# prstrive/SuRF

Measured on AMD Instinct MI355X. Metric: rays/sec (576x800, 5-view, 128 samp/ray render, whole job), higher is better.
Workload: dtype f32 (operands split exactly into 3 bf16 pieces, fp32 accumulate)

## Files before the change

surf_amd/csrc/sdf_mlp_split.hip:

```cpp
#include <math.h>
#include <stdlib.h>
#include <string.h>

#include "common.h"

#include "sdf_split_common.h"

namespace {

#ifdef SURF_SDF_TIMING
__device__ unsigned long long g_phase[8];
#define SURF_T(k)                                                 \
  do {                                                            \
    const unsigned long long now_ = __builtin_readcyclecounter(); \
    c.tacc[k] += now_ - c.tprev;                                  \
    c.tprev = now_;                                               \
  } while (0)
#else
#define SURF_T(k)
#endif

struct Ctx {
#ifdef SURF_SDF_TIMING
  mutable unsigned long long tprev;
  mutable unsigned long long tacc[8];
#endif
  rsrc_t wr, sr, sl, tr;
  int lane, lane16, h, svoff, wave;
  int wave1024;
  int dma_voff;
  uint32_t dma_lds;
  char* lds;
  char* lds_s;
  u32x4 I0, I1;
};
__device__ __forceinline__ u32x4 minus_identity_frag(int lane, int s) {
  const int i = lane & 31, g = lane >> 5;
  u32x4 f = {0u, 0u, 0u, 0u};
#pragma unroll
  for (int ip = 0; ip < 8; ++ip) {
    const int rho = (ip & 3) + 8 * (2 * s + (ip >> 2)) + 4 * g;
    if (rho == i) f[ip >> 1] |= (ip & 1) ? 0xBF800000u : 0x0000BF80u;
  }
  return f;
}
template <class P>
__device__ __forceinline__ void mres_step(const Ctx& c, f32x16& vt, const u32x4& piece, int s2) {
  if constexpr (P::MRES) {
    __builtin_amdgcn_sched_barrier(0);
    const u32x4 I = s2 ? c.I1 : c.I0;
    vt = __builtin_amdgcn_mfma_f32_32x32x16_bf16(__builtin_bit_cast(bf16x8, I), __builtin_bit_cast(bf16x8, piece), vt, 0, 0, 0);
    asm volatile("" ::"v"(vt));
    __builtin_amdgcn_sched_barrier(0);
  }
}

template <class P> constexpr int n_dma(int ci) { return (P::CH.ks[ci] * P::NP + 3) / 4; }
#ifndef SURF_SDF_DMA_WAVEMAJOR
#define SURF_SDF_DMA_WAVEMAJOR 1
#endif
template <class P, int NS, int CI, int k>
__device__ __forceinline__ void stage_dma_piece(const Ctx& c) {
  constexpr int OFF = P::CH.off[CI];
#if SURF_SDF_DMA_WAVEMAJOR
  constexpr int ND = n_dma<P>(CI);
  const uint32_t wshare = (uint32_t)c.wave1024 * (uint32_t)ND;
  __builtin_amdgcn_raw_ptr_buffer_load_lds(
      c.wr, (__attribute__((address_space(3))) void*)(uintptr_t)(c.dma_lds + wshare + ((CI % NS) * slot_bytes<P>() + (k >> 2) * 4096)), 16,
      c.lane16, (int)wshare + (OFF + (k >> 2) * 4096), (k & 3) * 1024, 0);
#else
  __builtin_amdgcn_raw_ptr_buffer_load_lds(
      c.wr, (__attribute__((address_space(3))) void*)(uintptr_t)(c.dma_lds + ((CI % NS) * slot_bytes<P>() + k * 4096)), 16, c.dma_voff,
      OFF + k * 4096, 0, 0);
#endif
}
template <class P, int NS, int CI, int K = 0>
__device__ __forceinline__ void stage_dma(const Ctx& c) {
  if constexpr (K < n_dma<P>(CI)) {
    stage_dma_piece<P, NS, CI, K>(c);
    stage_dma<P, NS, CI, K + 1>(c);
  }
}
constexpr int sprime_layer(bool deep, int L, int T, bool r0 = false) {
  if (!deep) return (L >= 1 && T < 4) ? L - 1 : -1;
  if (L >= 1 && T < 3) return L - 1;
  if (r0 && L == 2 && T == BWD_NT[L] - 1) return -1;
  if (L >= 2 && T == BWD_NT[L] - 1) return L - 2;
  return -1;
}
constexpr int sprime_tile(bool deep, int L, int T) { return !deep ? T : ((L >= 1 && T < 3) ? T + 1 : 0); }
template <class P> constexpr int lds_slice(int layer, int tile) {
  const int k = (4 - layer) * 4 + tile;
  return (layer <= 4 && layer >= 0 && k < P::LDS_SLICES) ? k : -1;
}
template <class P> constexpr int reg_slice(int layer, int tile) {
  const int k = (4 - layer) * 4 + tile - P::LDS_SLICES;
  return (layer <= 4 && layer >= 0 && k >= 0 && k < P::REG_SLICES) ? k : -1;
}
template <class P> constexpr bool on_chip(int layer, int tile) {
  return lds_slice<P>(layer, tile) >= 0 || reg_slice<P>(layer, tile) >= 0 || (P::R0 && layer == 0);
}
template <class P> struct RegSlices {
  f32x4 v[P::REG_SLICES > 0 ? P::REG_SLICES : 1][4];
  f32x16 r0[P::R0 ? 4 : 1];
};
constexpr int sprime_groups(int layer, int tile) { return (layer == 2 && tile == 3) ? 2 : 4; }
template <class P> constexpr int vm_pre(int ci) {
  if (ci < N_FWD_CHUNKS) return (ci / 4 == 5 && ci % 4 > 0) ? 4 : 0;
  if (ci >= P::CH.n) return 0;
  if (P::R0 && ci == r0_chunk()) return 0;
  int l = 5, t = ci - N_FWD_CHUNKS - ((P::R0 && ci > r0_chunk()) ? 1 : 0);
  while (t >= BWD_NT[l]) { t -= BWD_NT[l]; --l; }
  if (l == 0) return P::DEEPJ ? 12 : 0;
  if (sprime_layer(P::DEEP, l, t, P::R0) < 0 || on_chip<P>(sprime_layer(P::DEEP, l, t, P::R0), sprime_tile(P::DEEP, l, t))) return 0;
  return sprime_groups(sprime_layer(P::DEEP, l, t, P::R0), sprime_tile(P::DEEP, l, t));
}
template <class P, bool GRAD> constexpr int vm_post(int ci) {
  if (!GRAD || ci >= N_FWD_CHUNKS) return 0;
  const int l = ci / 4, t = ci % 4;
  if ((l == 0 && t == 0) || (l == 5 && t > 0)) return 0;
  return on_chip<P>(t == 0 ? l - 1 : l, t == 0 ? 3 : t - 1) ? 0 : 4;
}
template <class P, bool GRAD, int CI, int NCH>
constexpr int barrier_vmcnt() {
  constexpr int DIST = P::nslot(GRAD) - 1;
  int n = 0;
  for (int j = 0; j + 1 < DIST; ++j) {
    const int cj = (CI - j + NCH) % NCH;
    n += vm_pre<P>(cj) + n_dma<P>((cj + DIST) % NCH) + vm_post<P, GRAD>(cj);
  }
  return n;
}
template <class P, bool GRAD, int CI, int NCH>
__device__ __forceinline__ void stage_barrier() {
  constexpr int N = barrier_vmcnt<P, GRAD, CI, NCH>();
  static_assert(N >= 0 && N < 64, "vmcnt");
  asm volatile("; surf_ring_window %1\n\ts_waitcnt vmcnt(%0) lgkmcnt(0)\n\ts_barrier" ::"n"(N), "n"(P::nslot(GRAD) - 2) : "memory");
}

template <class P, bool GRAD, int CI, int NCH, class PL, int NACC, class BSel, class F>
__device__ __forceinline__ void run_chunk_n(const Ctx& c, BSel bsel, F slot, f32x16 (&result)[NACC]) {
  constexpr int NKS = P::CH.ks[CI];
  constexpr int NP = P::NP, NM = P::NM;
  constexpr int NS = P::nslot(GRAD);
  constexpr int KPA = NKS > 0 ? NKS / NACC : 1;
  static_assert(NKS % NACC == 0, "k-steps per accumulator");
  const char* rd = c.lds + (CI % NS) * slot_bytes<P>() + c.lane16;
  typename P::Acc accs[NACC];
#pragma unroll
  for (int a = 0; a < NACC; ++a)
#pragma unroll
    for (int q = 0; q < P::NA; ++q)
#pragma unroll
      for (int r = 0; r < 16; ++r) accs[a].v[q][r] = 0.f;
  constexpr int PF = P::PF;
  static_assert(PF == 1, "the gap plan places the reads of k-step ks + 1 behind the MFMAs of k-step ks");
  u32x4 a_q[PF + 1][NP];
#pragma unroll
  for (int d = 0; d < PF; ++d)
#pragma unroll
    for (int p = 0; p < NP; ++p)
      if (d < NKS) a_q[d][p] = *reinterpret_cast<const u32x4*>(rd + (d * NP + p) * 1024);
  constexpr int NXT = (CI + NS - 1) % NCH, ND = n_dma<P>(NXT);
  static_assert(ND <= MAX_DMA && NKS * NM <= MAX_GAPS, "GapPlan sizes");
// ... 252 lines not shown
  mini_add_split(mp, P::NP, P::FUSED_SUB, P::MRES);
  return mp;
}
template <class P, int L, int T, bool CONVERT>
struct BwdPlan {
  static constexpr int CI = bwd_chunk(L, T, P::R0), NKS = P::CH.ks[CI];
  static constexpr MiniProg mini = bwd_prog<P>();
  static constexpr SlotProg prog = CONVERT ? weave(mini, 8, 0, P::MRES ? P::NP : 0) : SlotProg{};
  static constexpr GapPlan v = plan_gaps(NKS, P::NM, P::NP, chunk_dma<P, true, CI, n_chunks<P>(true)>(), NKS * P::NM, prog);
  static_assert(plan_ok(v, prog, mini, NKS * P::NM, NKS * P::NM), "gap plan");
};
template <class P, int L, int T, bool CONVERT>
__device__ __forceinline__ f32x16 bwd_tile(const Ctx& c, const FragT<P::NP>* din, FragT<P::NP>* dout, const BwdPend& prev,
                                           f32x4 (&s_load)[4], const RegSlices<P>& keep) {
  typedef FragT<P::NP> Frag;
  typedef BwdPlan<P, L, T, CONVERT> PL;
  constexpr int CI = bwd_chunk(L, T, P::R0);
  constexpr int SL = sprime_layer(P::DEEP, L, T, P::R0);
  constexpr int NG = SL >= 0 ? sprime_groups(SL, sprime_tile(P::DEEP, L, T)) : 0;
  static_assert((SL >= 0 && on_chip<P>(SL, sprime_tile(P::DEEP, L, T)) ? 0 : NG) + ((L == 0 && P::DEEPJ) ? 12 : 0) == vm_pre<P>(CI),
                "vmcnt bookkeeping");
  if (SL >= 0) load_sprime<P, NG>(c, SL, sprime_tile(P::DEEP, L, T), s_load, keep);
  MiniState<P::NP> st[2] = {};
  f32x16 vt = prev.G;
  auto slot = [&](auto sc) __attribute__((always_inline)) {
    constexpr int s = decltype(sc)::value;
    constexpr float inv_w = 1.0f / Scales<P>::W;
    constexpr int q = PL::prog.q[s] < 0 ? 0 : PL::prog.q[s], kind = PL::prog.kind[s], i = PL::prog.arg[s], el = 2 * q;
    MiniState<P::NP>& S = st[q & 1];
    if constexpr (kind == K_EXPN) {
      const f32x2 u = {prev.s[el >> 2][el & 3], prev.s[(el + 1) >> 2][(el + 1) & 3]};
      S.e[0] = SURF_X_NOSOFTPLUS ? u[0] : __builtin_amdgcn_exp2f(-u[0]);
      S.e[1] = SURF_X_NOSOFTPLUS ? u[1] : __builtin_amdgcn_exp2f(-u[1]);
      slot_pin(S.e);
    } else if constexpr (kind == K_ADD1) {
      slot_pin(S.e);
      S.d[0] = S.e[0] + 1.0f;
      S.d[1] = S.e[1] + 1.0f;
      slot_pin(S.d);
    } else if constexpr (kind == K_RCP) {
      slot_pin(S.d);
      S.r[0] = SURF_X_NOSOFTPLUS ? S.d[0] : __builtin_amdgcn_rcpf(S.d[0]);
      S.r[1] = SURF_X_NOSOFTPLUS ? S.d[1] : __builtin_amdgcn_rcpf(S.d[1]);
      slot_pin(S.r);
    } else if constexpr (kind == K_MULG) {
      slot_pin(S.r);
      S.val[0] = S.r[0] * (P::MRES ? vt[el] : prev.G[el]);
      S.val[1] = S.r[1] * (P::MRES ? vt[el + 1] : prev.G[el + 1]);
      if (inv_w != 1.0f) {
        S.val[0] *= inv_w;
        S.val[1] *= inv_w;
      }
      slot_pin(S.val);
    } else if constexpr (kind == K_PACK) {
      slot_pin(S.val);
      S.pc[i] = SURF_X_NOSPLIT ? __builtin_bit_cast(uint32_t, S.val[i & 1]) : P::pack(S.val);
      slot_pin(S.pc[i]);
      if (P::MRES) {
        dout[2 * (T - 1) + (el >> 3)].p[0][(el & 7) >> 1] = S.pc[0];
        vt[el] = S.val[0];
        vt[el + 1] = S.val[1];
      } else if (i == P::NP - 1) {
        Frag& f = dout[2 * (T - 1) + (el >> 3)];
#pragma unroll
        for (int k = 0; k < P::NP; ++k) f.p[k][(el & 7) >> 1] = S.pc[k];
      }
    } else if constexpr (kind == K_MRES) {
      mres_step<P>(c, vt, dout[2 * (T - 1) + (i & 1)].p[i >> 1], i & 1);
    } else if constexpr (kind == K_PACKT) {
      const f32x2 r2 = {vt[el], vt[el + 1]};
      dout[2 * (T - 1) + (el >> 3)].p[i][(el & 7) >> 1] = P::pack(r2);
    } else if constexpr (kind == K_EXPAND) {
      slot_pin(S.pc[i]);
      S.x = SURF_X_NOSPLIT ? S.val : P::expand(S.pc[i]);
      slot_pin(S.x);
    } else if constexpr (kind == K_SUB) {
      slot_pin(S.val, S.x);
      S.val[0] -= S.x[0];
      S.val[1] -= S.x[1];
      slot_pin(S.val);
    } else if constexpr (kind == K_SUBP) {
      S.val = SURF_X_NOSPLIT ? S.val : P::sub_piece(S.val, S.pc[i]);
    }
  };
  return run_chunk<P, true, CI, n_chunks<P>(true), PL>(
      c, [&](int ks) __attribute__((always_inline)) -> const Frag& { return din[ks]; }, slot);
}
template <class P, int L, int T>
__device__ __forceinline__ void bwd_hidden_tile(const Ctx& c, const FragT<P::NP>* din, FragT<P::NP>* dout, BwdPend& pend, const RegSlices<P>& keep) {
  const BwdPend prev = pend;
  f32x4 s_load[4] = {};
  const f32x16 G = bwd_tile<P, L, T, (T > 0)>(c, din, dout, prev, s_load, keep);
  pend.G = G;
#pragma unroll
  for (int g = 0; g < 4; ++g) {
    if (P::DEEP) {
      pend.s[g] = prev.sn[g];
      pend.sn[g] = s_load[g];
    } else {
      pend.s[g] = s_load[g];
    }
  }
}
template <class P, int L>
__device__ __forceinline__ void bwd_layer(const Ctx& c, const FragT<P::NP>* din, FragT<P::NP>* dout, f32x16& accE,
                                          f32x16& accP, BwdPend& pend, const RegSlices<P>& keep) {
  bwd_hidden_tile<P, L, 0>(c, din, dout, pend, keep);
  bwd_hidden_tile<P, L, 1>(c, din, dout, pend, keep);
  bwd_hidden_tile<P, L, 2>(c, din, dout, pend, keep);
  bwd_hidden_tile<P, L, 3>(c, din, dout, pend, keep);
  const BwdPend prev = pend;
  if constexpr (L == 3) {
    f32x4 unused[4];
    accE += bwd_tile<P, L, 4, true>(c, din, dout, prev, unused, keep);
    accP += bwd_tile<P, L, 5, false>(c, din, dout, prev, pend.sn, keep);
  } else {
    accP += bwd_tile<P, L, 4, true>(c, din, dout, prev, pend.sn, keep);
  }
}

template <class P, int CI>
struct R0Plan {
  static constexpr GapPlan v = plan_gaps(R0_KS, P::NM, P::NP, chunk_dma<P, true, CI, n_chunks<P>(true)>(), R0_KS * P::NM, SlotProg{});
};
template <class P>
__device__ __forceinline__ void recompute_layer0(const Ctx& c, const FragT<P::NP> (&ef)[2], RegSlices<P>& keep) {
  if constexpr (P::R0) {
    constexpr int CI = r0_chunk();
    static_assert(P::CH.ks[CI] == R0_KS && P::CH.off[CI] == P::CH.off[fwd_chunk(0, 0)] && fwd_ne(0) == 2 && fwd_nl(0) == 2, "R0 chunk");
    run_chunk_n<P, true, CI, n_chunks<P>(true), R0Plan<P, CI>, 4>(
        c, [&](int ks) __attribute__((always_inline)) -> const FragT<P::NP>& { return ef[ks & 1]; }, [&](auto) __attribute__((always_inline)) {},
        keep.r0);
  }
}

template <class P, int CI>
struct PadPlan {
  static constexpr GapPlan v = plan_gaps(0, P::NM, P::NP, chunk_dma<P, true, CI, n_chunks<P>(true)>(), 0, SlotProg{});
};
template <class P, int CI>
__device__ __forceinline__ void pad_chunks(const Ctx& c, const FragT<P::NP>* any) {
  if constexpr (CI < n_chunks<P>(true)) {
    run_chunk<P, true, CI, n_chunks<P>(true), PadPlan<P, CI>>(
        c, [&](int ks) __attribute__((always_inline)) -> const FragT<P::NP>& { return any[0]; }, [&](auto) __attribute__((always_inline)) {});
    pad_chunks<P, CI + 1>(c, any);
  }
}

template <class P, bool GRAD, bool BRICK = false>
__global__ __launch_bounds__(WPB * 64, P::occ(GRAD)) void sdf_mlp_split_kernel(SdfArgs a) {
  typedef FragT<P::NP> Frag;
  constexpr int NS = P::nslot(GRAD), NCH = n_chunks<P>(GRAD);
  constexpr int NSL = GRAD ? P::LDS_SLICES : 0;
  __shared__ __attribute__((aligned(16))) char lds[NS * slot_bytes<P>() + WPB * NSL * 4096];
  static_assert(NCH % NS == 0 && (!GRAD || NCH - P::CH.n <= MAX_PAD) && NS >= 3, "slot of a chunk = index % ring length");
  Ctx c;
  c.lane = threadIdx.x & 63;
  c.wave = __builtin_amdgcn_readfirstlane(threadIdx.x >> 6);
  c.h = c.lane >> 5;
  c.lane16 = c.lane * 16;
  c.lds = lds;
  c.lds_s = lds + NS * slot_bytes<P>() + c.wave * (NSL * 4096) + c.lane16;
  if (P::MRES) {
    c.I0 = minus_identity_frag(c.lane, 0);
    c.I1 = minus_identity_frag(c.lane, 1);
  }
  c.wave1024 = c.wave * 1024;
  c.dma_voff = c.lane16 + c.wave * 1024;
  c.dma_lds = (uint32_t)(uintptr_t)(__attribute__((address_space(3))) char*)lds + (SURF_SDF_DMA_WAVEMAJOR ? 0 : c.wave * 1024);
  c.wr = __builtin_amdgcn_make_buffer_rsrc((void*)a.packed, 0, stream_bytes<P>(), 0x00020000);
  c.tr = __builtin_amdgcn_make_buffer_rsrc((void*)(a.packed + stream_bytes<P>()), 0, TAIL_FLOATS * 4, 0x00020000);
  c.sr = __builtin_amdgcn_make_buffer_rsrc((void*)a.scratch, 0, (GRAD && !(SURF_X_NOSCRATCH & 1)) ? 0x7fffffff : 0, 0x00020000);
  c.sl = __builtin_amdgcn_make_buffer_rsrc((void*)a.scratch, 0, (GRAD && !(SURF_X_NOSCRATCH & 2)) ? 0x7fffffff : 0, 0x00020000);
  const int64_t wave_id = (int64_t)blockIdx.x * WPB + c.wave;
  c.svoff = (int)(wave_id * (SCR_SLOT * 4)) + c.lane * 16;
  const int64_t n_pts = a.n_dev ? (int64_t)*a.n_dev : a.n;
  const int64_t n_tiles = (n_pts + TILE - 1) / TILE;
  const int64_t n_rounds = (n_tiles + WPB - 1) / WPB;

  stage_dma<P, NS, 0>(c);
  stage_dma<P, NS, 1>(c);
  if (NS > 3) stage_dma<P, NS, 2>(c);
  if (NS > 4) stage_dma<P, NS, 3>(c);
  asm volatile("s_waitcnt vmcnt(0) lgkmcnt(0)\n\ts_barrier" ::: "memory");
#ifdef SURF_SDF_TIMING
  c.tprev = __builtin_readcyclecounter();
  for (int k = 0; k < 8; ++k) c.tacc[k] = 0;
#endif
  for (int64_t round = blockIdx.x; round < n_rounds; round += gridDim.x) {
    asm volatile("" : "+s"(c.dma_lds));
    asm volatile("" : "+s"(c.wave1024));
    const int64_t tile = round * WPB + c.wave;
    const int64_t slot0 = tile * TILE + (c.lane & 31);
    const int64_t sc = slot0 < n_pts ? slot0 : n_pts - 1;
    int64_t i;
    bool active;
    float px, py, pz;
    if constexpr (BRICK) {
      i = sc;
      const uint32_t id = (uint32_t)a.idx[sc >> 9], l = (uint32_t)sc & 511u, nb = (uint32_t)a.lat_nz, last = (uint32_t)a.lat_ny - 1u;
      const uint32_t gx = id / (nb * nb) * 8u + (l >> 6), gy = id / nb % nb * 8u + ((l >> 3) & 7u), gz = id % nb * 8u + (l & 7u);
      active = (slot0 < n_pts) && gx <= last && gy <= last && gz <= last;
      px = a.lat_axes[0][gx < last ? gx : last];
      py = a.lat_axes[1][gy < last ? gy : last];
      pz = a.lat_axes[2][gz < last ? gz : last];
    } else {
      i = a.idx ? (int64_t)a.idx[sc] : sc;
      active = (slot0 < n_pts) && (!a.mask || a.mask[i] != 0);
      if (a.pts) {
        px = a.pts[i * 3 + 0]; py = a.pts[i * 3 + 1]; pz = a.pts[i * 3 + 2];
      } else {
        const uint32_t ii = (uint32_t)i, yz = ii / (uint32_t)a.lat_nz;
        px = a.lat_axes[0][yz / (uint32_t)a.lat_ny];
        py = a.lat_axes[1][yz % (uint32_t)a.lat_ny];
        pz = a.lat_axes[2][ii % (uint32_t)a.lat_nz];
      }
    }

    Frag ef[2], pf[2];
    float y0 = 0.f;
    SinCos3 base;
    {
      float phi[16];
      auto posenc = [&]() __attribute__((always_inline)) {
        float e[16], je_unused[14];
        base = sincos3(px, py, pz);
        posenc_half(c.h, px, py, pz, base, e, je_unused, false);
        e[14] = 1.0f;
        local_frags<P>(e, ef);
      };
      if (SURF_X_NOGATHER) {
#pragma unroll
        for (int ch = 0; ch < 16; ++ch) phi[ch] = px * (float)ch;
        posenc();
      } else {
        gather_features<GRAD>(a, c, px, py, pz, phi, posenc);
      }
      f32x4 w6p[4];
#pragma unroll
      for (int g = 0; g < 4; ++g) w6p[g] = bload(c.tr, c.h * 64, TAIL_W6P * 4 + g * 16);
#pragma unroll
      for (int g = 0; g < 4; ++g)
#pragma unroll
        for (int q = 0; q < 4; ++q)
          if (4 * g + q < 14) y0 = fmaf(w6p[g][q], phi[4 * g + q], y0);
      phi[14] = 1.0f;
      local_frags<P>(phi, pf);
    }
    SURF_T(0);

    Frag hA[8], hB[8], dA[8];
    RegSlices<P> keep;
    f32x16 raw;
#pragma unroll
    for (int r = 0; r < 16; ++r) raw[r] = 0.f;
    fwd_layer<P, GRAD, 0>(c, raw, hA, hA, ef, pf, dA, y0, keep);
    fwd_layer<P, GRAD, 1>(c, raw, hA, hB, ef, pf, dA, y0, keep);
    fwd_layer<P, GRAD, 2>(c, raw, hB, hA, ef, pf, dA, y0, keep);
    fwd_layer<P, GRAD, 3>(c, raw, hA, hB, ef, pf, dA, y0, keep);
    fwd_layer<P, GRAD, 4>(c, raw, hB, hA, ef, pf, dA, y0, keep);
    fwd_layer<P, GRAD, 5>(c, raw, hA, hB, ef, pf, dA, y0, keep);
    SURF_T(1);
    {
      f32x4 w6t[4];
#pragma unroll
      for (int g = 0; g < 4; ++g) w6t[g] = bload(c.tr, c.h * 256, TAIL_W6H * 4 + (12 + g) * 16);
#pragma unroll
      for (int g = 0; g < 4; ++g) {
        const f32x4 w = w6t[g];
        f32x2 hv[2], sv[2];
#pragma unroll
        for (int q = 0; q < 2; ++q) {
          const f32x2 t2 = {raw[4 * g + 2 * q], raw[4 * g + 2 * q + 1]};
          softplus_pair<GRAD ? 1 : 0, P::PRESCALED>(t2, 1.0f / Scales<P>::W, hv[q], sv[q]);
          y0 = fmaf(w[2 * q], hv[q][0], y0);
          y0 = fmaf(w[2 * q + 1], hv[q][1], y0);
          if (GRAD)
            frag_set_pair<P>(dA[6 + (g >> 1)], 2 * (g & 1) + q, sv[q][0] * (w[2 * q] * Scales<P>::D),
                             sv[q][1] * (w[2 * q + 1] * Scales<P>::D));
        }
      }
    }
    {
      const f32x4 b6 = bload(c.tr, 0, TAIL_B6 * 4);
      y0 += __shfl_xor(y0, 32);
      y0 += b6[0];
    }
    if (active && c.h == 0) a.sdf[i] = GRAD ? y0 : y0 * a.out_sign;
    SURF_T(2);
    if (GRAD) {
      f32x16 accE, accP;
#pragma unroll
      for (int r = 0; r < 16; ++r) accE[r] = 0.f;
      {
        f32x4 w[4];
#pragma unroll
        for (int g = 0; g < 4; ++g) w[g] = bload(c.tr, c.h * 64, TAIL_W6P * 4 + g * 16);
#pragma unroll
        for (int g = 0; g < 4; ++g)
#pragma unroll
          for (int q = 0; q < 4; ++q) accP[4 * g + q] = w[g][q] * (Scales<P>::W * Scales<P>::D);
      }
      BwdPend pend = {};
      if (P::DEEP) load_sprime<P>(c, 4, 0, pend.sn, keep);
      bwd_layer<P, 5>(c, dA, hA, accE, accP, pend, keep);
      bwd_layer<P, 4>(c, hA, dA, accE, accP, pend, keep);
      bwd_layer<P, 3>(c, dA, hA, accE, accP, pend, keep);
      bwd_layer<P, 2>(c, hA, dA, accE, accP, pend, keep);
      if constexpr (P::R0) {
        recompute_layer0<P>(c, ef, keep);
        load_sprime<P>(c, 0, 0, pend.sn, keep);
      }
      bwd_layer<P, 1>(c, dA, hA, accE, accP, pend, keep);
      f32x4 Jq[12];
      if (P::DEEPJ) {
#pragma unroll
        for (int g = 0; g < 12; ++g) Jq[g] = bload_scratch(c.sl, c.svoff, SCR_S * 4 + g * 1024);
      }
      {
        f32x4 unused[4];
        accE += bwd_tile<P, 0, 0, false>(c, hA, dA, pend, unused, keep);
      }
      pad_chunks<P, P::CH.n>(c, hA);
      SURF_T(3);
      float g3[3] = {0.f, 0.f, 0.f};
      {
        float e2[16], je[14];
        posenc_half(c.h, px, py, pz, base, e2, je, true);
#pragma unroll
        for (int s2 = 0; s2 < 14; ++s2) {
          const int c0 = s2 % 3, c1 = (14 + s2) % 3;
          const float v = accE[s2] * je[s2];
#pragma unroll
          for (int ax = 0; ax < 3; ++ax) g3[ax] += ((c.h ? c1 : c0) == ax) ? v : 0.f;
        }
#pragma unroll
        for (int sl = 0; sl < 2; ++sl) {
          float Jf[24];
#pragma unroll
          for (int g = 0; g < 6; ++g) {
            const f32x4 v = P::DEEPJ ? Jq[6 * sl + g] : bload_scratch(c.sl, c.svoff, SCR_S * 4 + (6 * sl + g) * 1024);
            Jf[4 * g + 0] = v[0]; Jf[4 * g + 1] = v[1]; Jf[4 * g + 2] = v[2]; Jf[4 * g + 3] = v[3];
          }
#pragma unroll
          for (int ch = 0; ch < 7; ++ch) {
#pragma unroll
            for (int ax = 0; ax < 3; ++ax) g3[ax] = fmaf(accP[7 * sl + ch], Jf[3 * ch + ax], g3[ax]);
          }
        }
      }
#pragma unroll
      for (int ax = 0; ax < 3; ++ax) g3[ax] = (g3[ax] + __shfl_xor(g3[ax], 32)) * (1.0f / (Scales<P>::W * Scales<P>::D));
      if (active && c.h == 0) {
        a.grad[i * 3 + 0] = g3[0];
        a.grad[i * 3 + 1] = g3[1];
        a.grad[i * 3 + 2] = g3[2];
      }
      SURF_T(4);
    }
  }
  asm volatile("s_waitcnt vmcnt(0)" ::: "memory");
#ifdef SURF_SDF_TIMING
  if (threadIdx.x == 0)
    for (int k = 0; k < 8; ++k) atomicAdd(&g_phase[k], c.tacc[k]);
#endif
}

template <class P>
int grid_blocks(int64_t n, bool grad) {
  int64_t tiles = (n + TILE - 1) / TILE;
  int64_t rounds = (tiles + WPB - 1) / WPB;
  return (int)(rounds < max_blocks<P>(grad) ? rounds : max_blocks<P>(grad));
}

inline uint16_t bf16_rne(float f) {
  uint32_t u;
  memcpy(&u, &f, 4);
  if ((u & 0x7fffffffu) > 0x7f800000u) return (uint16_t)((u >> 16) | 0x40);
  u += 0x7fffu + ((u >> 16) & 1u);
  return (uint16_t)(u >> 16);
}
inline float bf16_to_f(uint16_t b) {
  uint32_t u = (uint32_t)b << 16;
  float f;
  memcpy(&f, &u, 4);
  return f;
}
inline uint16_t f16_bits(float v) {
  _Float16 h = (_Float16)v;
  uint16_t b;
  memcpy(&b, &h, 2);
  return b;
}
inline float f16_to_f(uint16_t b) {
  _Float16 h;
  memcpy(&h, &b, 2);
  return (float)h;
}
template <class P> void split_host(float v, uint16_t* p);
template <> void split_host<PolBf3>(float v, uint16_t* p) {
  p[0] = bf16_rne(v);
  float r = v - bf16_to_f(p[0]);
  p[1] = bf16_rne(r);
  r = r - bf16_to_f(p[1]);
  p[2] = bf16_rne(r);
}
template <> void split_host<PolH2>(float v, uint16_t* p) {
  p[0] = f16_bits(v);
  p[1] = f16_bits(v - f16_to_f(p[0]));
}
inline int frag_feat(int tt, int s, int j, int h) { return 32 * tt + 16 * s + (j & 3) + 8 * (j >> 2) + 4 * h; }

template <class P>
int pack_weights(const float* const* h_W, const float* const* h_b, unsigned char* out) {
  if (!h_W || !h_b || !out) return SURF_E_ARG;
  for (int l = 0; l < 7; ++l)
    if (!h_W[l] || !h_b[l]) return SURF_E_ARG;
  constexpr int NP = P::NP;
  const int in_dim[7] = {NE, 156, 156, 156, 156, 156, 156};
  const int out_dim[6] = {HID, HID, H2, HID, HID, HID};
  const float rsqrt2 = (float)(1.0 / sqrt(2.0));
  const float c_in = P::PRESCALED ? (float)(100.0 * 1.4426950408889634) : 1.0f;
  const float c_in_rsqrt2 = P::PRESCALED ? (float)(100.0 * 1.4426950408889634 / sqrt(2.0)) : rsqrt2;
  const float k_out = P::PRESCALED ? (float)(0.6931471805599453 / 100.0) : 1.0f;
  memset(out, 0, stream_bytes<P>() + TAIL_FLOATS * 4);
  auto put = [&](int chunk, int ks, int lane, int j, float v) {
    uint16_t p[NP];
    split_host<P>(v * Scales<P>::W, p);
    for (int pc = 0; pc < NP; ++pc) {
      uint16_t* dst = reinterpret_cast<uint16_t*>(out + P::CH.off[chunk] + (ks * NP + pc) * 1024 + lane * 16);
      dst[j] = p[pc];
    }
  };
  for (int l = 0; l < 6; ++l)
    for (int t = 0; t < 4; ++t) {
      const int ci = fwd_chunk(l, t);
      const int hid_in = (l == 3) ? H2 : HID;
      for (int ks = 0; ks < fwd_ks(l); ++ks)
        for (int lane = 0; lane < 64; ++lane)
          for (int j = 0; j < 8; ++j) {
            const int h = lane >> 5, row = 32 * t + (lane & 31);
            int col = -1;
            float scale = 1.f;
            bool is_bias = false;
            if (ks < fwd_ne(l)) {
              const int cidx = 8 * ks + j;
              if (cidx < 14 && 14 * h + cidx < NE) col = (l == 3 ? H2 : 0) + 14 * h + cidx;
              scale = l == 3 ? c_in_rsqrt2 : c_in;
              if (l == 0) is_bias = (cidx == 14 && h == 0);
            } else if (ks < fwd_nl(l)) {
              const int cidx = 8 * (ks - fwd_ne(l)) + j;
              if (cidx < 14) col = 128 + 14 * h + cidx;
              scale = c_in;
              is_bias = (cidx == 14 && h == 0);
            } else {
              const int hk = ks - fwd_nl(l);
              const int f = frag_feat(hk >> 1, hk & 1, j, h);
              if (f < hid_in) col = f;
              if (l == 3) scale = rsqrt2;
            }
            float v = 0.f;
            if (col >= 0 && row < out_dim[l]) v = h_W[l][(int64_t)row * in_dim[l] + col] * scale;
            if (is_bias && row < out_dim[l]) v = h_b[l][row] * c_in;
            put(ci, ks, lane, j, v);
          }
    }
  for (int l = 0; l < 6; ++l)
    for (int t = 0; t < BWD_NT[l]; ++t) {
      const int ci = bwd_chunk(l, t, P::R0);
      const int hid_in = (l == 3) ? H2 : HID;
      for (int ks = 0; ks < bwd_ks(l); ++ks)
        for (int lane = 0; lane < 64; ++lane)
          for (int j = 0; j < 8; ++j) {
            const int h = lane >> 5, rho = lane & 31;
            const int krow = frag_feat(ks >> 1, ks & 1, j, h);
            const int h_row = (rho >> 2) & 1, r_row = (rho & 3) | ((rho >> 3) << 2);
            const int ch = 14 * h_row + r_row;
            int kind;
            if (l == 0) kind = 1;
            else if (t < 4) kind = 0;
            else if (l == 3 && t == 4) kind = 1;
            else kind = 2;
            int col = -1;
            float scale = 1.f;
            if (kind == 0) {
              const int cc = 32 * t + rho;
              if (cc < hid_in) col = cc;
              if (l == 3) scale = rsqrt2;
            } else if (kind == 1) {
              if (r_row < 14 && ch < NE) col = (l == 3 ? H2 : 0) + ch;
              scale = l == 3 ? c_in_rsqrt2 : c_in;
            } else {
              if (r_row < 14) col = 128 + ch;
              scale = c_in;
            }
            float v = 0.f;
            if (col >= 0 && krow < out_dim[l]) v = h_W[l][(int64_t)krow * in_dim[l] + col] * scale;
            put(ci, ks, lane, j, v);
          }
    }
  float* tail = reinterpret_cast<float*>(out + stream_bytes<P>());
  auto hk = [](int tt, int r, int h) { return 32 * tt + (r & 3) + 8 * (r >> 2) + 4 * h; };
  for (int h = 0; h < 2; ++h) {
    for (int s = 0; s < 64; ++s) tail[TAIL_W6H + h * 64 + s] = h_W[6][hk(s / 16, s % 16, h)] * k_out;
    for (int s = 0; s < 14; ++s) tail[TAIL_W6P + h * 16 + s] = h_W[6][128 + 14 * h + s];
  }
  tail[TAIL_B6] = h_b[6][0];
  return 0;
}

struct Lattice { const float* ax[3]; int ny, nz; float sign; bool bricks; };
template <class P>
int launch(const float* pts, const uint8_t* mask, const int32_t* idx, int64_t n, const float* const* h_vols,
           const int32_t* const* h_tables, const int* h_dims, int n_vol, const void* packed, float* sdf, float* grad,
           void* scratch, void* stream, const int32_t* d_n, const Lattice* lat = nullptr) {
  if ((!pts && !lat) || !h_vols || !h_tables || !h_dims || !packed || !sdf) return SURF_E_ARG;
  if (n <= 0 || n_vol <= 0) return SURF_E_ARG;
  if (n_vol > SURF_MAX_STAGES) return SURF_E_LIMIT;
  if (grad && !scratch) return SURF_E_ARG;
  SdfArgs a;
  a.pts = pts; a.mask = mask; a.idx = idx; a.n = n; a.n_dev = d_n; a.packed = (const unsigned char*)packed; a.sdf = sdf; a.grad = grad;
  a.scratch = (float*)scratch;
  a.lat_axes[0] = a.lat_axes[1] = a.lat_axes[2] = nullptr; a.lat_ny = a.lat_nz = 1; a.out_sign = 1.0f;
  if (lat) {
    if (grad || mask || (idx != nullptr) != lat->bricks || d_n || n >= (int64_t)1 << 31 || lat->ny < 1 || lat->nz < 1 || !lat->ax[0] || !lat->ax[1] || !lat->ax[2]) return SURF_E_ARG;
    for (int k = 0; k < 3; ++k) a.lat_axes[k] = lat->ax[k];
    a.lat_ny = lat->ny; a.lat_nz = lat->nz; a.out_sign = lat->sign;
    if (lat->bricks) a.idx = idx;
  }
  for (int s = 0; s < SURF_MAX_STAGES; ++s) {
    a.vols[s] = s < n_vol ? h_vols[s] : h_vols[0];
    a.tables[s] = s < n_vol ? h_tables[s] : h_tables[0];
    a.dims[s] = s < n_vol ? h_dims[s] : 0;
    if (s < n_vol && (!h_vols[s] || !h_tables[s] || h_dims[s] <= 1)) return SURF_E_ARG;
    if (s < n_vol && h_dims[s] > 1024) return SURF_E_LIMIT;
  }
  dim3 grid(grid_blocks<P>(n, grad != nullptr)), block(WPB * 64);
  if (lat && lat->bricks)
    hipLaunchKernelGGL((sdf_mlp_split_kernel<P, false, true>), grid, block, 0, (hipStream_t)stream, a);
  else if (grad)
    hipLaunchKernelGGL((sdf_mlp_split_kernel<P, true>), grid, block, 0, (hipStream_t)stream, a);
  else
    hipLaunchKernelGGL((sdf_mlp_split_kernel<P, false>), grid, block, 0, (hipStream_t)stream, a);
  return surf_check_launch();
}

template <class P>
int launch_lattice(const float* ax, const float* ay, const float* az, int nx, int ny, int nz, const float* const* h_vols,
                   const int32_t* const* h_tables, const int* h_dims, int n_vol, const void* packed, float* out, float sign, void* stream) {
  if (nx < 1 || ny < 1 || nz < 1) return SURF_E_ARG;
  const Lattice lat = {{ax, ay, az}, ny, nz, sign, false};
  return launch<P>(nullptr, nullptr, nullptr, (int64_t)nx * ny * nz, h_vols, h_tables, h_dims, n_vol, packed, out, nullptr, nullptr, stream,
                   nullptr, &lat);
}

template <class P>
int launch_bricks(const float* ax, const float* ay, const float* az, int res, const int32_t* bricks, int64_t n_bricks,
                  const float* const* h_vols, const int32_t* const* h_tables, const int* h_dims, int n_vol, const void* packed, float* out,
                  float sign, void* stream) {
  if (res < 2 || res > SURF_BAND_MAX_RES || !bricks || n_bricks <= 0) return SURF_E_ARG;
  if (n_bricks * 512 >= (int64_t)1 << 31) return SURF_E_LIMIT;
  const Lattice lat = {{ax, ay, az}, res, (res + 7) / 8, sign, true};
  return launch<P>(nullptr, nullptr, bricks, n_bricks * 512, h_vols, h_tables, h_dims, n_vol, packed, out, nullptr, nullptr, stream,
                   nullptr, &lat);
}

template <class P>
int64_t scratch_bytes(int64_t n_points) {
  if (n_points <= 0) return 0;
  return (int64_t)grid_blocks<P>(n_points, true) * WPB * SCR_SLOT * sizeof(float);
}

}

#ifdef SURF_SDF_TIMING
#ifdef SURF_SDF_TU_F16
#define SURF_DEBUG_PHASES surf_debug_phases_f16
#else
#define SURF_DEBUG_PHASES surf_debug_phases
#endif
extern "C" int SURF_DEBUG_PHASES(unsigned long long* out, int reset) {
  if (hipMemcpyFromSymbol(out, HIP_SYMBOL(g_phase), sizeof(unsigned long long) * 8) != hipSuccess) return 100;
  if (reset) {
    unsigned long long z[8] = {0, 0, 0, 0, 0, 0, 0, 0};
    if (hipMemcpyToSymbol(HIP_SYMBOL(g_phase), z, sizeof(z)) != hipSuccess) return 100;
  }
  return 0;
}
#endif

#ifndef SURF_SDF_TU_F16

extern "C" int64_t surf_sdf_bf16_packed_bytes(void) { return stream_bytes<PolBf3>() + TAIL_FLOATS * 4; }
extern "C" int64_t surf_sdf_bf16_scratch_bytes(int64_t n_points) { return scratch_bytes<PolBf3>(n_points); }
extern "C" int surf_sdf_pack_weights_bf16(const float* const* h_W, const float* const* h_b, unsigned char* out) {
  return pack_weights<PolBf3>(h_W, h_b, out);
}
extern "C" int surf_sdf_mlp_bf16x3(const float* pts, const uint8_t* mask, const int32_t* idx, int64_t n,
                                   const float* const* h_vols, const int32_t* const* h_tables, const int* h_dims, int n_vol,
                                   const void* packed, float* sdf, float* grad, void* scratch, void* stream) {
  return launch<PolBf3>(pts, mask, idx, n, h_vols, h_tables, h_dims, n_vol, packed, sdf, grad, scratch, stream, nullptr);
}
extern "C" int surf_sdf_mlp_bf16x3_dn(const float* pts, const int32_t* idx, int64_t n_capacity, const int32_t* d_n,
                                     const float* const* h_vols, const int32_t* const* h_tables, const int* h_dims, int n_vol,
                                     const void* packed, float* sdf, float* grad, void* scratch, void* stream) {
  if (!idx || !d_n) return SURF_E_ARG;
  return launch<PolBf3>(pts, nullptr, idx, n_capacity, h_vols, h_tables, h_dims, n_vol, packed, sdf, grad, scratch, stream, d_n);
}

extern "C" int surf_sdf_lattice_bf16x3(const float* ax, const float* ay, const float* az, int nx, int ny, int nz, const float* const* h_vols,
                                       const int32_t* const* h_tables, const int* h_dims, int n_vol, const void* packed, float* out,
                                       float sign, void* stream) {
  return launch_lattice<PolBf3>(ax, ay, az, nx, ny, nz, h_vols, h_tables, h_dims, n_vol, packed, out, sign, stream);
}
extern "C" int surf_sdf_bricks_bf16x3(const float* ax, const float* ay, const float* az, int res, const int32_t* bricks, int64_t n_bricks,
                                      const float* const* h_vols, const int32_t* const* h_tables, const int* h_dims, int n_vol,
                                      const void* packed, float* out, float sign, void* stream) {
  return launch_bricks<PolBf3>(ax, ay, az, res, bricks, n_bricks, h_vols, h_tables, h_dims, n_vol, packed, out, sign, stream);
}

#else
extern "C" int surf_sdf_lattice_f16x2(const float* ax, const float* ay, const float* az, int nx, int ny, int nz, const float* const* h_vols,
                                      const int32_t* const* h_tables, const int* h_dims, int n_vol, const void* packed, float* out,
                                      float sign, void* stream) {
  return launch_lattice<PolH2>(ax, ay, az, nx, ny, nz, h_vols, h_tables, h_dims, n_vol, packed, out, sign, stream);
}
extern "C" int surf_sdf_bricks_f16x2(const float* ax, const float* ay, const float* az, int res, const int32_t* bricks, int64_t n_bricks,
                                     const float* const* h_vols, const int32_t* const* h_tables, const int* h_dims, int n_vol,
                                     const void* packed, float* out, float sign, void* stream) {
  return launch_bricks<PolH2>(ax, ay, az, res, bricks, n_bricks, h_vols, h_tables, h_dims, n_vol, packed, out, sign, stream);
}
extern "C" int64_t surf_sdf_f16_packed_bytes(void) { return stream_bytes<PolH2>() + TAIL_FLOATS * 4; }
extern "C" int64_t surf_sdf_f16_scratch_bytes(int64_t n_points) { return scratch_bytes<PolH2>(n_points); }
extern "C" int surf_sdf_pack_weights_f16(const float* const* h_W, const float* const* h_b, unsigned char* out) {
  return pack_weights<PolH2>(h_W, h_b, out);
}
extern "C" int surf_sdf_mlp_f16x2(const float* pts, const uint8_t* mask, const int32_t* idx, int64_t n,
                                  const float* const* h_vols, const int32_t* const* h_tables, const int* h_dims, int n_vol,
                                  const void* packed, float* sdf, float* grad, void* scratch, void* stream) {
  return launch<PolH2>(pts, mask, idx, n, h_vols, h_tables, h_dims, n_vol, packed, sdf, grad, scratch, stream, nullptr);
}
extern "C" int surf_sdf_mlp_f16x2_dn(const float* pts, const int32_t* idx, int64_t n_capacity, const int32_t* d_n,
                                    const float* const* h_vols, const int32_t* const* h_tables, const int* h_dims, int n_vol,
                                    const void* packed, float* sdf, float* grad, void* scratch, void* stream) {
  if (!idx || !d_n) return SURF_E_ARG;
  return launch<PolH2>(pts, nullptr, idx, n_capacity, h_vols, h_tables, h_dims, n_vol, packed, sdf, grad, scratch, stream, d_n);
}
#endif
```

surf_amd/csrc/sdf_split_common.h:

```cpp
#pragma once
#include <math.h>
#include <stdlib.h>
#include <string.h>

#include "common.h"

namespace {


constexpr int HID = 128, NE = 27, H2 = 101, TILE = 32;
constexpr int BWD_NT[6] = {1, 5, 5, 6, 5, 5};
constexpr int WPB = 4;
constexpr int MAX_KS = 12;

constexpr int fwd_nh(int l) { return l == 0 ? 0 : (l == 3 ? 7 : 8); }
constexpr int fwd_ne(int l) { return (l == 0 || l == 3) ? 2 : 0; }
constexpr int fwd_np(int l) { return l == 0 ? 0 : 2; }
constexpr int fwd_nl(int l) { return fwd_ne(l) + fwd_np(l); }
constexpr int fwd_ks(int l) { return fwd_nh(l) + fwd_nl(l); }
constexpr int bwd_ks(int l) { return l == 2 ? 7 : 8; }
constexpr int N_FWD_CHUNKS = 24;
constexpr int n_bwd_chunks() { int n = 0; for (int l = 0; l < 6; ++l) n += BWD_NT[l]; return n; }
constexpr int N_BWD_CHUNKS = n_bwd_chunks();
constexpr int N_CHUNKS = N_FWD_CHUNKS + N_BWD_CHUNKS;
// ... 84 lines not shown
#ifndef SURF_X_NOSPLIT
#define SURF_X_NOSPLIT 0
#endif

#ifndef SURF_SDF_NSLOT_BF3
#define SURF_SDF_NSLOT_BF3 3
#endif
#ifndef SURF_SDF_NSLOT_H2
#define SURF_SDF_NSLOT_H2 3
#endif

#ifndef SURF_SDF_LDS_SLICES_BF3
#define SURF_SDF_LDS_SLICES_BF3 3
#endif
#ifndef SURF_SDF_LDS_SLICES_H2
#define SURF_SDF_LDS_SLICES_H2 5
#endif
#ifndef SURF_SDF_REG_SLICES_BF3
#define SURF_SDF_REG_SLICES_BF3 9
#endif
#ifndef SURF_SDF_REG_SLICES_H2
#define SURF_SDF_REG_SLICES_H2 15
#endif

struct PolBf3 {
#ifndef SURF_SDF_NA_BF3
#define SURF_SDF_NA_BF3 1
#endif
  static constexpr int NP = 3, NA = SURF_SDF_NA_BF3, PF = 1;
  static constexpr int occ(bool) { return 1; }
  static constexpr int nslot(bool) { return SURF_SDF_NSLOT_BF3; }
  static constexpr int REG_SLICES = SURF_SDF_REG_SLICES_BF3;
  static constexpr int LDS_SLICES = SURF_SDF_LDS_SLICES_BF3;
#ifndef SURF_SDF_DEEP_BF3
#define SURF_SDF_DEEP_BF3 1
#endif
  static constexpr bool DEEP = SURF_SDF_DEEP_BF3;
  static constexpr bool DEEPJ = true;
#ifndef SURF_SDF_R0_BF3
#define SURF_SDF_R0_BF3 1
#endif
  static constexpr bool R0 = SURF_SDF_R0_BF3;
  static constexpr ChunkTable CH = make_chunks(NP, R0);
  struct Acc { f32x16 v[NA]; };
  static __device__ __forceinline__ uint32_t pack2(float a, float b) {
    bf16x2 v;
    v[0] = (__bf16)a;
    v[1] = (__bf16)b;
    uint32_t u = __builtin_bit_cast(uint32_t, v);
    asm volatile("" : "+v"(u));
    return u;
  }
  static __device__ __forceinline__ void split(float a, float b, uint32_t (&p)[NP]) { surf_split3_bf16(a, b, p); }
  static __device__ __forceinline__ uint32_t pack(f32x2 v) { return pack2(v[0], v[1]); }
  static __device__ __forceinline__ f32x2 expand(uint32_t p) {
    f32x2 x;
    x[0] = __builtin_bit_cast(float, p << 16);
    x[1] = __builtin_bit_cast(float, p & 0xffff0000u);
    return x;
  }
  static constexpr bool FUSED_SUB = false;
#ifndef SURF_SDF_MRES_BF3
#define SURF_SDF_MRES_BF3 0
#endif
  static constexpr bool MRES = SURF_SDF_MRES_BF3;
  static constexpr bool PRESCALED = true;
  static __device__ __forceinline__ f32x2 sub_piece(f32x2 v, uint32_t p) { return v - expand(p); }
  static constexpr int NM = 6;
  static __device__ __forceinline__ void mma_one(Acc& acc, const u32x4 (&a)[NP], const FragT<NP>& b, int m) {
    constexpr int X[6] = {2, 0, 1, 1, 0, 0}, Y[6] = {0, 2, 1, 0, 1, 0};
    acc.v[m & (NA - 1)] = __builtin_amdgcn_mfma_f32_32x32x16_bf16(__builtin_bit_cast(bf16x8, a[X[m]]), __builtin_bit_cast(bf16x8, b.p[Y[m]]),
                                                                 acc.v[m & (NA - 1)], 0, 0, 0);
  }
  static __device__ __forceinline__ void mma(Acc& acc, const u32x4 (&a)[NP], const FragT<NP>& b) {
#pragma unroll
    for (int m = 0; m < NM; ++m) mma_one(acc, a, b, m);
  }
  static __device__ __forceinline__ f32x16 finish(const Acc& acc) {
    if (NA == 1) return acc.v[0];
    f32x16 r;
#pragma unroll
    for (int i = 0; i < 16; ++i) r[i] = acc.v[0][i] + acc.v[NA - 1][i];
    return r;
  }
};

struct PolH2 {
  static constexpr int NP = 2, NA = 1, PF = 1;
  static constexpr int occ(bool grad) { return grad ? 1 : 2; }
  static constexpr int nslot(bool grad) { return grad ? SURF_SDF_NSLOT_H2 : 3; }
  static constexpr int REG_SLICES = SURF_SDF_REG_SLICES_H2;
  static constexpr int LDS_SLICES = SURF_SDF_LDS_SLICES_H2;
  static constexpr bool DEEP = true, DEEPJ = true;
  static constexpr bool R0 = false;
  static constexpr ChunkTable CH = make_chunks(NP, R0);
  struct Acc { f32x16 v[NA]; };
  static __device__ __forceinline__ void split(float a, float b, uint32_t (&p)[NP]) {
    const f32x2 v = {a, b};
    const f16x2 h = __builtin_convertvector(v, f16x2);
    const f32x2 r = v - __builtin_convertvector(h, f32x2);
    p[0] = __builtin_bit_cast(uint32_t, h);
    p[1] = __builtin_bit_cast(uint32_t, __builtin_convertvector(r, f16x2));
  }
  static __device__ __forceinline__ uint32_t pack(f32x2 v) {
    uint32_t p = __builtin_bit_cast(uint32_t, __builtin_convertvector(v, f16x2));
    asm volatile("" : "+v"(p));
    return p;
  }
  static __device__ __forceinline__ f32x2 expand(uint32_t p) { return __builtin_convertvector(__builtin_bit_cast(f16x2, p), f32x2); }
  static constexpr bool FUSED_SUB = true;
  static constexpr bool MRES = false;
  static constexpr bool PRESCALED = false;
  static __device__ __forceinline__ f32x2 sub_piece(f32x2 v, uint32_t p) {
    f32x2 r;
    asm("v_fma_mix_f32 %0, %1, -1.0, %2 op_sel:[0,0,0] op_sel_hi:[1,0,0]" : "=v"(r[0]) : "v"(p), "v"(v[0]));
    asm("v_fma_mix_f32 %0, %1, -1.0, %2 op_sel:[1,0,0] op_sel_hi:[1,0,0]" : "=v"(r[1]) : "v"(p), "v"(v[1]));
    return r;
  }
  static constexpr int NM = 3;
  static __device__ __forceinline__ void mma_one(Acc& acc, const u32x4 (&a)[NP], const FragT<NP>& b, int m) {
    constexpr int X[3] = {1, 0, 0}, Y[3] = {0, 1, 0};
    acc.v[0] = __builtin_amdgcn_mfma_f32_32x32x16_f16(__builtin_bit_cast(f16x8, a[X[m]]), __builtin_bit_cast(f16x8, b.p[Y[m]]), acc.v[0], 0, 0, 0);
  }
  static __device__ __forceinline__ void mma(Acc& acc, const u32x4 (&a)[NP], const FragT<NP>& b) {
#pragma unroll
    for (int m = 0; m < NM; ++m) mma_one(acc, a, b, m);
  }
  static __device__ __forceinline__ f32x16 finish(const Acc& acc) { return acc.v[0]; }
};

template <class P> struct Scales { static constexpr float W = 1.0f, D = 1.0f; };
template <> struct Scales<PolH2> { static constexpr float W = 256.0f, D = 256.0f; };

template <class P> constexpr int stream_bytes() { return P::CH.total; }
template <class P> constexpr int slot_bytes() { return MAX_KS * P::NP * 1024; }
template <class P> constexpr int max_blocks(bool grad) { return 256 * P::occ(grad); }
template <class P> constexpr int n_chunks(bool grad) {
  return grad ? (P::CH.n + P::nslot(true) - 1) / P::nslot(true) * P::nslot(true) : N_FWD_CHUNKS;
}

struct SdfArgs {
  const float* pts;
  const uint8_t* mask;
  const int32_t* idx;
  int64_t n;
  const int32_t* n_dev;
  const float* vols[SURF_MAX_STAGES];
  const int32_t* tables[SURF_MAX_STAGES];
  int dims[SURF_MAX_STAGES];
  const unsigned char* packed;
  float* sdf;
  float* grad;
  float* scratch;
  const float* lat_axes[3];
  int lat_ny, lat_nz;
  float out_sign;
};

__device__ __forceinline__ f32x4 bload(rsrc_t r, int voff, int soff) {
  return __builtin_bit_cast(f32x4, __builtin_amdgcn_raw_buffer_load_b128(r, voff, soff, 0));
}
#ifndef SURF_X_SCRATCH_NT
#define SURF_X_SCRATCH_NT 0
#endif
__device__ __forceinline__ f32x4 bload_scratch(rsrc_t r, int voff, int soff) {
  return __builtin_bit_cast(f32x4, __builtin_amdgcn_raw_buffer_load_b128(r, voff, soff, (SURF_X_SCRATCH_NT & 2) ? 2 : 0));
}
__device__ __forceinline__ void bstore(rsrc_t r, int voff, int soff, f32x4 v) {
#if SURF_X_SCRATCH_NT & 1
  asm volatile("buffer_store_dwordx4 %0, %1, %2, %3 offen nt\n\ts_nop 1" ::"v"(v), "v"(voff), "s"(r), "s"(soff) : "memory");
#else
  asm volatile("buffer_store_dwordx4 %0, %1, %2, %3 offen\n\ts_nop 1" ::"v"(v), "v"(voff), "s"(r), "s"(soff) : "memory");
#endif
}

template <class P>
__device__ __forceinline__ void frag_set_pair(FragT<P::NP>& f, int pair , float a, float b) {
  uint32_t p[P::NP];
  if (SURF_X_NOSPLIT) {
#pragma unroll
    for (int k = 0; k < P::NP; ++k) p[k] = __builtin_bit_cast(uint32_t, k & 1 ? a : b);
  } else {
    P::split(a, b, p);
  }
#pragma unroll
  for (int k = 0; k < P::NP; ++k) f.p[k][pair] = p[k];
}

template <int MODE, bool PRESCALED = false>
__device__ __forceinline__ void softplus_pair(f32x2 acc, float acc_scale_inv, f32x2& hv, f32x2& sv) {
  if (SURF_X_NOSOFTPLUS) {
    hv = acc * acc_scale_inv;
    sv = acc * 0.5f;
    return;
  }
  const f32x2 arg = PRESCALED ? acc : acc * (144.269504088896341f * acc_scale_inv);
  f32x2 e;
  e[0] = __builtin_amdgcn_exp2f(-__builtin_fabsf(arg[0]));
  e[1] = __builtin_amdgcn_exp2f(-__builtin_fabsf(arg[1]));
  const f32x2 d = e + 1.0f;
  f32x2 l;
  l[0] = __builtin_amdgcn_logf(d[0]);
  l[1] = __builtin_amdgcn_logf(d[1]);
  f32x2 m;
  m[0] = __builtin_amdgcn_fmed3f(acc[0], 0.0f, 3.0e38f);
  m[1] = __builtin_amdgcn_fmed3f(acc[1], 0.0f, 3.0e38f);
  if (acc_scale_inv != 1.0f) m = m * acc_scale_inv;
  if (PRESCALED) {
    hv = m + l;
  } else {
    hv[0] = fmaf(l[0], 0.69314718055994531f * 0.01f, m[0]);
    hv[1] = fmaf(l[1], 0.69314718055994531f * 0.01f, m[1]);
  }
  if (MODE == 1) {
    f32x2 r, sel;
    r[0] = __builtin_amdgcn_rcpf(d[0]);
    r[1] = __builtin_amdgcn_rcpf(d[1]);
    sel[0] = acc[0] >= 0.0f ? 1.0f : e[0];
    sel[1] = acc[1] >= 0.0f ? 1.0f : e[1];
    sv = sel * r;
  } else if (MODE == 2) {
    sv = arg;
  }
}

enum MiniKind : int {
  K_ARG, K_EXP, K_ADD1, K_LOG, K_MAX, K_FMA,
  K_Y0, K_RCP, K_SEL, K_SIG,
  K_EXPN, K_MULG,
  K_PACK, K_EXPAND, K_SUB,
  K_SUBP,
  K_MRES,
  K_PACKT
};
constexpr int MAX_MINI = 24, MAX_SLOTS = 8 * MAX_MINI;
struct MiniProg { int n; int kind[MAX_MINI]; int arg[MAX_MINI]; int cost[MAX_MINI]; };
constexpr void mini_add(MiniProg& mp, int kind, int arg, int cost) {
  mp.kind[mp.n] = kind; mp.arg[mp.n] = arg; mp.cost[mp.n] = cost; ++mp.n;
}
constexpr void mini_add_split(MiniProg& mp, int np, bool fused_sub, bool mres = false) {
  if (mres) {
    mini_add(mp, K_PACK, 0, 4);
    return;
  }
  for (int i = 0; i < np; ++i) {
    mini_add(mp, K_PACK, i, 4);
    if (i + 1 < np && fused_sub) mini_add(mp, K_SUBP, i, 8);
    if (i + 1 < np && !fused_sub) { mini_add(mp, K_EXPAND, i, 8); mini_add(mp, K_SUB, i, 8); }
  }
}
struct SlotProg { int n; int q[MAX_SLOTS]; int j[MAX_SLOTS]; int cost[MAX_SLOTS]; int kind[MAX_SLOTS]; int arg[MAX_SLOTS]; int per_pair; };
constexpr SlotProg weave(MiniProg mp, int pairs, int store_cost, int mres_np = 0) {
  SlotProg sp{};
  const int per = (pairs / 2) * mp.n, lag = mp.n | 1;
  int ia = 0, ib = 0;
  while (ia < per || ib < per) {
    const bool take_a = ib >= per || (ia < per && 2 * ia <= 2 * ib + lag);
    const int i = take_a ? ia++ : ib++;
    const int q = 2 * (i / mp.n) + (take_a ? 0 : 1), j = i % mp.n;
    sp.q[sp.n] = q; sp.j[sp.n] = j;
    sp.kind[sp.n] = mp.kind[j]; sp.arg[sp.n] = mp.arg[j];
    sp.cost[sp.n] = mp.cost[j] + ((j == mp.n - 1 && (q & 1)) ? store_cost : 0);
    ++sp.n;
  }
  sp.per_pair = mp.n;
  for (int lvl = 1; lvl < mres_np; ++lvl) {
    for (int s2 = 0; s2 < 2; ++s2) {
      sp.q[sp.n] = -1; sp.j[sp.n] = 0; sp.kind[sp.n] = K_MRES; sp.arg[sp.n] = 2 * (lvl - 1) + s2; sp.cost[sp.n] = 0;
      ++sp.n;
    }
    for (int q = 0; q < pairs; ++q) {
      sp.q[sp.n] = q; sp.j[sp.n] = mp.n + lvl - 1; sp.kind[sp.n] = K_PACKT; sp.arg[sp.n] = lvl; sp.cost[sp.n] = 4;
      ++sp.n;
    }
    sp.per_pair = mp.n + lvl;
  }
  return sp;
}

constexpr int MAX_GAPS = MAX_KS * 6, MAX_DMA = 12;
struct GapPlan {
  int first[MAX_GAPS + 1];
  int dma_gap[MAX_DMA];
  int cap, per_stream;
};
constexpr GapPlan plan_gaps(int nks, int nm, int np, int n_dma, int deadline, SlotProg sp) {
  GapPlan pl{};
  const int ng = nks * nm;
  int fixed[MAX_GAPS + 1] = {};
  for (int ks = 0; ks + 1 < nks; ++ks)
    for (int m = 0; m < np && m < nm; ++m) fixed[ks * nm + m] += 8;
  for (int k = 0; k < n_dma; ++k) {
    int g = 0;
    if (ng > 0) g = n_dma <= nks ? ((k * nks) / n_dma) * nm + nm - 1 : (k * ng) / n_dma;
    pl.dma_gap[k] = g;
    fixed[g] += 12;
  }
  if (deadline > ng) deadline = ng;
  int at[MAX_SLOTS] = {};
  int cap = 24, per = 1;
  for (bool done = sp.n == 0; !done;) {
    for (cap = 24; cap <= 32 + 8 * per && !done; cap += 4) {
      int g = 0, used = fixed[0], cnt[2] = {0, 0};
      int mres_gap = -1;
      bool ok = true, after_mres = false;
      for (int s = 0; s < sp.n && ok; ++s) {
// ... 241 lines not shown
```

Before: 2.928 million.

## Schedule gradient SDF rounds dynamically via a global atomic work counter

Replaces the static grid-stride loop over rounds in the gradient SDF MLP kernel with dynamic work dealing. Thread 0 of each block atomically fetches the next round index, publishes it through a double-buffered LDS word, and all waves read it at the end of the iteration. The aim is to balance load across workgroups whose per-round cost varies, reducing tail imbalance at the cost of one global atomic per round and a small scratch prefix that must be zeroed with a memset before each launch. Timing builds also record per-workgroup start and end times and round counts.

```diff
diff --git a/surf_amd/csrc/sdf_mlp_split.hip b/surf_amd/csrc/sdf_mlp_split.hip
--- a/surf_amd/csrc/sdf_mlp_split.hip
+++ b/surf_amd/csrc/sdf_mlp_split.hip
@@ -8,8 +8,14 @@
 
 namespace {
 
+#ifndef SURF_SDF_DEAL
+#define SURF_SDF_DEAL 1
+#endif
+constexpr int DEAL_BYTES = 256;
+
 #ifdef SURF_SDF_TIMING
 __device__ unsigned long long g_phase[8];
+__device__ unsigned long long g_swg[256][4];
 #define SURF_T(k)                                                 \
   do {                                                            \
     const unsigned long long now_ = __builtin_readcyclecounter(); \
@@ -568,7 +574,9 @@
   typedef FragT<P::NP> Frag;
   constexpr int NS = P::nslot(GRAD), NCH = n_chunks<P>(GRAD);
   constexpr int NSL = GRAD ? P::LDS_SLICES : 0;
-  __shared__ __attribute__((aligned(16))) char lds[NS * slot_bytes<P>() + WPB * NSL * 4096];
+  constexpr bool DEAL = SURF_SDF_DEAL && GRAD && !BRICK;
+  constexpr int DEAL_LDS = NS * slot_bytes<P>() + WPB * NSL * 4096;
+  __shared__ __attribute__((aligned(16))) char lds[DEAL_LDS + (DEAL ? 16 : 0)];
   static_assert(NCH % NS == 0 && (!GRAD || NCH - P::CH.n <= MAX_PAD) && NS >= 3, "slot of a chunk = index % ring length");
   Ctx c;
   c.lane = threadIdx.x & 63;
@@ -602,8 +610,17 @@
 #ifdef SURF_SDF_TIMING
   c.tprev = __builtin_readcyclecounter();
   for (int k = 0; k < 8; ++k) c.tacc[k] = 0;
+  const unsigned long long rt_begin = __builtin_amdgcn_s_memrealtime();
+  unsigned long long rounds_done = 0;
 #endif
-  for (int64_t round = blockIdx.x; round < n_rounds; round += gridDim.x) {
+  uint32_t parity = 0;
+  for (int64_t round = blockIdx.x; round < n_rounds;) {
+    uint32_t dealt = 0;
+    if (DEAL && threadIdx.x == 0) {
+      uint32_t z = 0;
+      asm volatile("" : "+v"(z));
+      dealt = __hip_atomic_fetch_add(a.next_round + z, 1u, __ATOMIC_RELAXED, __HIP_MEMORY_SCOPE_AGENT);
+    }
     asm volatile("" : "+s"(c.dma_lds));
     asm volatile("" : "+s"(c.wave1024));
     const int64_t tile = round * WPB + c.wave;
@@ -663,6 +680,7 @@
       phi[14] = 1.0f;
       local_frags<P>(phi, pf);
     }
+    if (DEAL && threadIdx.x == 0) *reinterpret_cast<uint32_t*>(lds + DEAL_LDS + parity * 4) = dealt;
     SURF_T(0);
 
     Frag hA[8], hB[8], dA[8];
@@ -774,11 +792,26 @@
       }
       SURF_T(4);
     }
+#ifdef SURF_SDF_TIMING
+    ++rounds_done;
+#endif
+    if (DEAL) {
+      round = (int64_t)gridDim.x + (uint32_t)__builtin_amdgcn_readfirstlane(*reinterpret_cast<const uint32_t*>(lds + DEAL_LDS + parity * 4));
+      parity ^= 1u;
+    } else {
+      round += gridDim.x;
+    }
   }
   asm volatile("s_waitcnt vmcnt(0)" ::: "memory");
 #ifdef SURF_SDF_TIMING
   if (threadIdx.x == 0)
     for (int k = 0; k < 8; ++k) atomicAdd(&g_phase[k], c.tacc[k]);
+  if (GRAD && threadIdx.x == 0 && blockIdx.x < 256) {
+    g_swg[blockIdx.x][0] = rt_begin;
+    g_swg[blockIdx.x][1] = __builtin_amdgcn_s_memrealtime();
+    g_swg[blockIdx.x][2] = __builtin_amdgcn_s_getreg(20 | (0 << 6) | (3 << 11));
+    g_swg[blockIdx.x][3] = rounds_done;
+  }
 #endif
 }
 
@@ -952,6 +985,12 @@
     if (s < n_vol && h_dims[s] > 1024) return SURF_E_LIMIT;
   }
   dim3 grid(grid_blocks<P>(n, grad != nullptr)), block(WPB * 64);
+  a.next_round = nullptr;
+  if (grad && SURF_SDF_DEAL) {
+    a.next_round = (uint32_t*)scratch;
+    a.scratch = (float*)((char*)scratch + DEAL_BYTES);
+    if (hipError_t e = hipMemsetAsync(a.next_round, 0, sizeof(uint32_t), (hipStream_t)stream); e != hipSuccess) return (int)e;
+  }
   if (lat && lat->bricks)
     hipLaunchKernelGGL((sdf_mlp_split_kernel<P, false, true>), grid, block, 0, (hipStream_t)stream, a);
   else if (grad)
@@ -984,7 +1023,7 @@
 template <class P>
 int64_t scratch_bytes(int64_t n_points) {
   if (n_points <= 0) return 0;
-  return (int64_t)grid_blocks<P>(n_points, true) * WPB * SCR_SLOT * sizeof(float);
+  return (SURF_SDF_DEAL ? DEAL_BYTES : 0) + (int64_t)grid_blocks<P>(n_points, true) * WPB * SCR_SLOT * sizeof(float);
 }
 
 }
@@ -992,9 +1031,14 @@
 #ifdef SURF_SDF_TIMING
 #ifdef SURF_SDF_TU_F16
 #define SURF_DEBUG_PHASES surf_debug_phases_f16
+#define SURF_DEBUG_WG surf_debug_sdf_wg_f16
 #else
 #define SURF_DEBUG_PHASES surf_debug_phases
+#define SURF_DEBUG_WG surf_debug_sdf_wg
 #endif
+extern "C" int SURF_DEBUG_WG(unsigned long long* out) {
+  return hipMemcpyFromSymbol(out, HIP_SYMBOL(g_swg), sizeof(unsigned long long) * 1024) == hipSuccess ? 0 : 100;
+}
 extern "C" int SURF_DEBUG_PHASES(unsigned long long* out, int reset) {
   if (hipMemcpyFromSymbol(out, HIP_SYMBOL(g_phase), sizeof(unsigned long long) * 8) != hipSuccess) return 100;
   if (reset) {
diff --git a/surf_amd/csrc/sdf_split_common.h b/surf_amd/csrc/sdf_split_common.h
--- a/surf_amd/csrc/sdf_split_common.h
+++ b/surf_amd/csrc/sdf_split_common.h
@@ -260,6 +260,7 @@
   float* sdf;
   float* grad;
   float* scratch;
+  uint32_t* next_round;
   const float* lat_axes[3];
   int lat_ny, lat_nz;
   float out_sign;
```

Result: faster. 3.036 million, median of 6 (+3.7%).
